# philgzl/brever

Measured on AMD Instinct MI355X. Metric: utterances/sec (4 s @16 kHz) Conv-TasNet train, higher is better.
Workload: dtype bf16

## Files before the change

brever_amd/csrc/convtasnet.hip:

```cpp
#include <hip/hip_runtime.h>
#include <stdio.h>
#include <stdlib.h>
#include <string.h>
#include <algorithm>
#include <string>
#include <vector>

#include "../../include/brever_hip.h"
#include "status.h"
#include "ctn_layout.h"
#include "gemm_rows.cuh"
#include "gemm_wgrad.cuh"
#include "gemm_ws.cuh"
#include "dwpw2_fused.cuh"
#include "gemm_wgrad_full.cuh"
#include "gemm_wgrad_full128.cuh"

constexpr int kWgSplit = 4;
#include "prep.cuh"
#include "tcn_kernels.cuh"
#include "bwd_fused.cuh"
#include "pw1_bwd.cuh"
#include "cln_kernels.cuh"

using namespace brv;

namespace {

inline long long align_up(long long x, long long a) { return (x + a - 1)/a*a; }

const brv_launch_opts kDefaultOpts = {sizeof(brv_launch_opts), 0u, 8, 0, nullptr};
thread_local const brv_launch_opts* t_opts = &kDefaultOpts;
struct OptsScope {
  const brv_launch_opts* prev;
  explicit OptsScope(const brv_launch_opts* o) : prev(t_opts) {
    t_opts = (o && o->size >= sizeof(brv_launch_opts)) ? o : &kDefaultOpts;
  }
  ~OptsScope() { t_opts = prev; }
  int check() const {
    const uint32_t unknown = t_opts->flags & ~BRV_OPT_KNOWN;
    if (!unknown) return 0;
// ... 59 lines not shown
      blk[i].p_c1_b = ptake((long long)Bnp*Hp);
      blk[i].p_rs_f = ptake((long long)rs*Hp);
      blk[i].p_rs_b = ptake((long long)Hp*rs);
      blk[i].p_c1_fp = ptake((long long)Hp*Bnp);
      blk[i].p_rs_fp = ptake((long long)rs*Hp);
      blk[i].p_rs_bp = ptake((long long)Hp*rs);
      blk[i].p_rs_g = ptake((long long)(Bnp + Scp)*Hp);
      blk[i].p_rs_gp = ptake((long long)(Bnp + Scp)*Hp);
      blk[i].p_lazy = ptake(4LL*(Bnp + Scp));
    }
    p_out_f = ptake((long long)S*Np*Scp);
    p_out_b = ptake((long long)Scp*S*Np);
    p_stamp = ptake(128);
    n_prepared = q;
    return 0;
  }
};

struct Workspace {
  long long w, x, z1, z2, skip, m, y, stats, sums, dpre, dw1, gskip, gout, eA, eB,
      e0, dwt, vg, gcopy, total;
  long long gcopy_stride, eB_stride;
  long long wgpart;
  long long h1, h2, wn, ctab, ctab_stride, cfs, cbt, ident, fake_stats, scratch_stats;
  long long vg_stride, vg_bytes;
  long long x_stride, z_stride;
  long long u, u_stride;
  long long stamp;
  long long stats_bytes;
  void init(const Layout& l, long long B, long long T) {
    long long o = 0;
    auto take = [&](long long bytes) { long long r = o; o += align_up(bytes, 256); return r; };
    const long long BT = B*T;
    w = take(BT*l.Np*2);
    x_stride = align_up(BT*l.Bnp*2, 256);
    x = take(x_stride*l.nb);
    z_stride = align_up(BT*l.Hp*2, 256);
    z1 = take(z_stride*l.nb);
    z2 = take(z_stride*l.nb);
    skip = take(BT*l.Scp*4);
    m = take(BT*l.S*l.Np*2);
    y = take(BT*l.S*l.Np*2);
    stats_bytes = (long long)(1 + 2*l.nb)*B*kStatStride*8;
    stats = take(stats_bytes);
    sums = take(stats_bytes);
    dpre = take(BT*l.S*l.Np*2);
    dw1 = take(BT*l.S*l.Np*2);
    gout = take(BT*(l.Bnp + l.Scp)*2);
    gskip = gout + (long long)l.Bnp*2;
    eA = take(BT*l.Hp*2);
    eB_stride = align_up(BT*l.Hp*2, 256);
    eB = take(eB_stride*l.nb);
    gcopy_stride = align_up(BT*l.Bnp*2, 256);
    gcopy = take(gcopy_stride*l.nb);
    e0 = take(BT*l.Np*2);
    dwt = take(BT*l.Np*2);
    vg_stride = align_up(2LL*l.N + (long long)l.nb*l.H*(5 + l.P) + 1 + 2*l.nb + 2LL*l.Hp, 64);
    vg_bytes = vg_stride*kReplicas*4;
    vg = take(vg_bytes);
    wgpart = take((long long)2*kWgSplit*l.nb*W2_G*l.H*4);
    u_stride = align_up(BT*(l.Bnp + l.Scp)*2, 256);
    u = l.fusable() ? take(u_stride*l.nb) : 0;
    stamp = take(256);
    h1 = h2 = wn = ctab = cfs = cbt = ident = fake_stats = scratch_stats = 0; ctab_stride = 0;
    if (l.causal) {
      h1 = take(z_stride*l.nb);
      h2 = take(z_stride*l.nb);
      wn = take(BT*l.Np*2);
      ctab_stride = align_up(BT*2*4, 256);
      ctab = take(ctab_stride*(1 + 2*l.nb));
      cfs = take(BT*2*4);
      cbt = take(BT*2*4);
      const long long cmax = l.Hp > l.Np ? l.Hp : l.Np;
      ident = take((2*cmax + 64)*4);
      fake_stats = take(B*kStatStride*8);
      scratch_stats = take(B*kStatStride*8);
    }
    total = o;
  }
};

struct Views {
  const Layout& l; Workspace ws; char* base; const bf16_t* prep; int B; long long T;
// ... 174 lines not shown
  if (p.Kp % GR_BK != 0 || p.Np % 64 != 0) return fail(-1, "gemm_rows: unpadded dims");
  if (p.Np % 128 == 0) return launch_gemm_rows_t<128, AK, EM>(p, batch, st);
  return launch_gemm_rows_t<64, AK, EM>(p, batch, st);
}

inline int wgrad_target(const char* label, int dflt) {
  (void)label;
  return t_opts->wg_target != 0 ? t_opts->wg_target : dflt;
}

template <int BH, int HK>
int launch_wgrad_t(WgradGroupParams& gp, hipStream_t st, int target) {
  WgradParams& p = gp.base;
  const int nprob = gp.nprob > 0 ? gp.nprob : 1;
  const int tiles = ceil_div(p.Gp, WG_BG)*(p.Hp/BH);
  const int total = p.B*ceil_div(p.T, WG_BT);
  int ns = ceil_div(target > 0 ? target : 384, tiles*nprob);
  if (target < 0) {
    int nb = p.B;
    while (tiles*nprob*nb > 2048 && nb % 2 == 0) nb /= 2;
    if (nb > ns) ns = nb;
  }
  if (ns > total) ns = total;
  if (ns < 1) ns = 1;
  p.nsplit = ns;
  dim3 grid(tiles, ns, nprob);
  hipLaunchKernelGGL((gemm_wgrad_kernel<BH, HK>), grid, dim3(256), 0, st, gp);
  BRV_HIP_OK(hipGetLastError());
  return 0;
}
template <int HK>
int launch_wgrad_group(WgradGroupParams& gp, hipStream_t st, const char* label,
                       double bytes, int target_dflt = 384) {
  const WgradParams& p = gp.base;
  if (p.T <= 0 || p.B <= 0) return 0;
  const int nprob = gp.nprob > 0 ? gp.nprob : 1;
  ProfScope prof(label, 2.0*nprob*p.B*p.T*(double)p.Gp*p.Hp, bytes*nprob, st);
  if (p.Hp % 64 != 0) return fail(-1, "wgrad: unpadded dims");
  const int target = wgrad_target(label, target_dflt);
  if (p.Hp % 128 == 0) return launch_wgrad_t<128, HK>(gp, st, target);
  return launch_wgrad_t<64, HK>(gp, st, target);
}
template <int HK>
int launch_wgrad(WgradParams& p, hipStream_t st, const char* label = "wgrad",
                 double bytes = 0, int target_dflt = 384) {
  WgradGroupParams gp;
  gp.base = p; gp.nprob = 0;
  return launch_wgrad_group<HK>(gp, st, label, bytes, target_dflt);
}

template <template <int> class F, typename... Args>
int dispatch_p(int P, Args&&... args) {
  switch (P) {
    case 1: return F<1>::run(args...);
    case 2: return F<2>::run(args...);
    case 3: return F<3>::run(args...);
    case 4: return F<4>::run(args...);
    case 5: return F<5>::run(args...);
  }
  return fail(-2, "unsupported kernel_size");
}
template <int P> struct DwFwd {
  static int run(const DwParams& p, hipStream_t st) {
    ProfScope prof("dwconv_fwd", 2.0*P*p.B*p.T*(double)p.Cp, 4.0*p.B*p.T*(double)p.Cp, st);
    dim3 grid(ceil_div(p.T, DW_TT_F)*p.B);
    hipLaunchKernelGGL((dwconv_fwd_kernel<P>), grid, dim3(256), 0, st, p);
    BRV_HIP_OK(hipGetLastError());
    return 0;
  }
};
template <int P> struct DwBwd {
// ... 49 lines not shown
  int gx = (int)((per_item + 256*8 - 1)/(256*8));
  const int cap = 1024/p.B > 1 ? 1024/p.B : 1;
  if (gx > cap) gx = cap;
  if (gx < 1) gx = 1;
  hipLaunchKernelGGL(dz_kernel, dim3(gx, p.B), dim3(256), 0, st, p);
  BRV_HIP_OK(hipGetLastError());
  return 0;
}

ASpec rows_bf16(const void* ptr, int ld, long long T) {
  ASpec a; memset(&a, 0, sizeof(a));
  a.p0 = ptr; a.ld0 = ld; a.bs0 = T*ld; a.K0 = 1 << 30; a.nsrc = 1;
  return a;
}
void set_affine(ASpec& a, const double* stats, const float* g, const float* b, int C,
                long long T) {
  a.stats = stats; a.gamma = g; a.beta = b; a.C = C;
  a.inv_n = 1.0/((double)T*(double)C); a.eps = 1e-8f;
}
ASpec frames_of(const float* wav, long long L, int hop, int K, long long stride = 0) {
  ASpec a; memset(&a, 0, sizeof(a));
  a.p0 = wav; a.hop = hop; a.Kf = K; a.wav_stride = stride > 0 ? stride : L; a.wav_len = (int)L;
  a.K0 = 1 << 30; a.nsrc = 1;
  return a;
}

struct PrepJobC { int src_off, dst_off, scale_off; unsigned short R, C, rows, cols, dst_ld, tr; };
constexpr int kPrepBatch = 168;
struct PrepBatch { PrepJobC jobs[kPrepBatch]; int n; };
static_assert(sizeof(PrepBatch) <= 4096, "kernel argument size");

struct PackJob { long long src_off, dst_off; int N, K, nsl; };
struct PackBatch { PackJob jobs[96]; int n; };
__global__ __launch_bounds__(256) void pack_frag_kernel(bf16_t* prepared, const PackBatch pb) {
  const PackJob j = pb.jobs[blockIdx.y];
  const long long total = (long long)j.N*j.K/8;
  const int KS = j.K/16;
  for (long long i = (long long)blockIdx.x*256 + threadIdx.x; i < total; i += (long long)gridDim.x*256) {
    const int n = (int)(i / (j.K/8)), k = (int)(i % (j.K/8))*8;
    const int slice = n / j.nsl, f = (n % j.nsl)/32, fr = n % 32, s = k/16, fh = (k % 16)/8;
    const long long dst = (long long)slice*j.nsl*j.K + ((long long)(f*KS + s)*64 + fr + 32*fh)*8;
    *reinterpret_cast<uint4*>(prepared + j.dst_off + dst) =
        *reinterpret_cast<const uint4*>(prepared + j.src_off + (long long)n*j.K + k);
  }
}
__global__ __launch_bounds__(256) void prep_weights_kernel(const float* params,
// ... 94 lines not shown
        float f[8];
        unpack8(q[k], f);
        const float r = rs[i + k];
#pragma unroll
        for (int j = 0; j < 8; ++j) acc[j] = __builtin_fmaf(r, f[j], acc[j]);
      }
    }
    for (; i < p.nb; ++i) {
      float f[8];
      unpack8(*reinterpret_cast<const uint4*>(src + i*p.u_stride), f);
      const float r = rs[i];
#pragma unroll
      for (int j = 0; j < 8; ++j) acc[j] = __builtin_fmaf(r, f[j], acc[j]);
    }
    float* dst = p.skip + ((long long)b*p.T + t)*p.Scp + c0;
    *reinterpret_cast<float4*>(dst) = make_float4(acc[0], acc[1], acc[2], acc[3]);
    *reinterpret_cast<float4*>(dst + 4) = make_float4(acc[4], acc[5], acc[6], acc[7]);
  }
}

}

int reduce_vector_grads(const Views& v, float* grads, hipStream_t st, int blk_lo = 0, int blk_hi = 1 << 30,
                        bool do_ln = true, bool do_tcn = true) {
  const Layout& l = v.l;
  const long long vper = (long long)l.H*(5 + l.P);
  {
    VgradParams vp; memset(&vp, 0, sizeof(vp));
    vp.vg = v.vg(); vp.grads = grads; vp.rep_stride = v.ws.vg_stride;
    vp.N = l.N; vp.H = l.H; vp.P = l.P; vp.nb = l.nb;
    vp.ln_g_off = l.ln_g; vp.blk0_off = l.blk[0].conv_w;
    vp.blk_full = l.nb > 1 ? l.blk[1].conv_w - l.blk[0].conv_w : 0;
    const BlockOff& b0 = l.blk[0];
    const BlockOff& bl = l.blk[l.nb - 1];
    vp.o_dconv_w = b0.dconv_w - b0.conv_w; vp.o_dconv_b = b0.dconv_b - b0.conv_w;
    vp.o_n1_g_full = b0.n1_g - b0.conv_w; vp.o_n1_g_last = bl.n1_g - bl.conv_w;
    vp.tcn_prelu_off = l.tcn_prelu;
    vp.blk_lo = blk_lo; vp.blk_hi = blk_hi; vp.do_ln = do_ln; vp.do_tcn = do_tcn;
    if (b0.prelu1 != b0.n1_g + 4LL*l.H || b0.prelu2 != b0.prelu1 + 1)
      return fail(-1, "vgrad_reduce: unexpected PReLU offsets");
    const long long total = 2LL*l.N + vper*l.nb + 1 + 2*l.nb;
    int gx = (int)((total + 255)/256);
    if (gx > 1024) gx = 1024;
    ProfScope prof("vgrad_reduce", 0, 4.0*total*(kReplicas + 2), st);
    hipLaunchKernelGGL(vgrad_reduce_kernel, dim3(gx), dim3(256), 0, st, vp);
    BRV_HIP_OK(hipGetLastError());
  }
  return 0;
}

__global__ void fill_identity_kernel(float* ones, float* zeros, float* one, int n,
                                     double* fake_stats, int B, double sumsq) {
  const int i = blockIdx.x*256 + threadIdx.x;
  if (i < n) { ones[i] = 1.f; zeros[i] = 0.f; }
  if (i == 0) *one = 1.f;
  if (i < B) { fake_stats[stat_sum(i)] = 0.0; fake_stats[stat_sq(i)] = sumsq; }
}

namespace {

int causal_init(const Views& v, hipStream_t st) {
  const Layout& l = v.l;
  const double sumsq = (1.0 - (double)1e-8f)*(double)v.T*(double)l.H;
  const int cmax = (int)v.cmax(), n = cmax > v.B ? cmax : v.B;
  hipLaunchKernelGGL(fill_identity_kernel, dim3((n + 255)/256), dim3(256), 0, st, v.ones(), v.zeros(),
                     v.one(), cmax, v.fake_stats(), v.B, sumsq);
  BRV_HIP_OK(hipGetLastError());
// ... 371 lines not shown
  }
  else
  if (int r = launch_wgrad_group<A_BF16>(gp, st, "pw1_wgrad", 2.0*BT*(l.Hp + l.Bnp), -1))
    return r;
  return 0;
}

int deferred_wgrads(const Views& v, const float* params, float* grads, int blk_lo, int blk_hi, hipStream_t st) {
  const Layout& l = v.l;
  const bool full_rs = l.Bnp == 128 && l.Scp == 128 && l.Hp % W2_BH == 0 && l.nb <= kWgMaxProb &&
                       !opt(BRV_OPT_NO_WGRAD_FULL);
  if (full_rs && blk_lo <= blk_hi)
    if (int r = wgrad_rs_full(v, params, grads, blk_lo, blk_hi, st)) return r;
  for (int i0 = blk_lo; i0 <= blk_hi; i0 += kWgMaxProb) {
    const int n = std::min(kWgMaxProb, blk_hi + 1 - i0);
    if (!full_rs)
      if (int r = wgrad_rs_grouped(v, params, grads, i0, n, st)) return r;
    if (int r = wgrad_pw1(v, params, grads, i0, n, st)) return r;
  }
  return 0;
}

int backward_head(const Views& v, const float* params, const float* d_out, float* grads, long long L,
                  bool bwd_fused, hipStream_t st) {
  const Layout& l = v.l; const int B = v.B; const long long T = v.T; const double BT = v.BT();
  const int BS = B*l.S, ldg = v.ldg(); GemmRowsParams g; WgradParams wg;
  if (!l.causal)
    if (int r = launch_call_init(v.sum(0), (long long)(v.ws.stats_bytes/8), v.vg(), (long long)v.ws.vg_bytes,
                                 reinterpret_cast<const int*>(v.base + v.ws.stamp), mode_stamp(l.fused_fwd()), nullptr, 0, st))
      return fail(r, "backward: call_init launch");
  memset(&g, 0, sizeof(g));
  g.a = frames_of(d_out, L, l.hop, l.K);
  g.W = v.prep + l.p_dec_b; g.T = (int)T; g.Np = l.Np; g.Kp = l.Kfp;
  g.e.out = v.dpre(); g.e.ldo = l.Np; g.e.out2 = v.dw1(); g.e.w_in = v.w(); g.e.ld_w = l.Np;
  g.e.m_in = v.m(); g.e.S = l.S;
  if (int r = launch_gemm_rows<A_FRAMES, E_MASK_BWD>(g, BS, st, "dec_bwd", 4.0*BS*L + 2.0*BT*l.Np*(1 + 3*l.S))) return r;
  memset(&wg, 0, sizeof(wg));
  wg.g = rows_bf16(v.y(), l.Np, T); wg.h = frames_of(d_out, L, l.hop, l.K);
  wg.B = BS; wg.T = (int)T; wg.Gp = l.Np; wg.Hp = l.Kfp;
  wg.out0 = grads + l.dec_w; wg.G0p = l.Np; wg.N0 = l.N; wg.Kout = l.K; wg.ldo = l.K;
  if (int r = launch_wgrad<A_FRAMES>(wg, st, "wgrad_dec", 2.0*BT*l.S*l.Np + 4.0*BS*L, l.causal ? 384 : 768)) return r;
  memset(&g, 0, sizeof(g));
  g.a = rows_bf16(v.dpre(), l.Np, T); g.a.nsrc = l.S;
  g.W = v.prep + l.p_out_b; g.T = (int)T; g.Np = l.Scp; g.Kp = l.S*l.Np;
  g.e.out = v.gskip(); g.e.ldo = ldg; g.e.src_f32 = v.skip(); g.e.ld_srcf = l.Scp;
  g.e.src_slope = params + l.tcn_prelu; g.e.dslope = v.vslope();
  g.e.rep_stride = v.ws.vg_stride; g.e.n_rep = kReplicas;
  if (int r = launch_gemm_rows<A_BF16, E_PRELU_BWD>(g, B, st, "mask_bwd", 2.0*BT*l.S*l.Np + 6.0*BT*l.Scp)) return r;
  if (bwd_fused) {
    GuDotsParams gu; memset(&gu, 0, sizeof(gu));
    gu.g = v.gskip(); gu.ldg = ldg; gu.u = v.u(l.nb - 1) + l.Bnp; gu.ldu = ldg;
    gu.v1 = reinterpret_cast<const float*>(v.prep + l.blk[l.nb - 1].p_lazy) + ldg + l.Bnp;
    gu.ncols = l.Scp; gu.B = B; gu.T = (int)T; gu.out = v.sum(2 + 2*(l.nb - 1));
    ProfScope prof("gu_dots", 0, 4.0*BT*l.Scp, st);
    int gx = (int)((T*(l.Scp/8) + 255)/256);
    if (gx > 64) gx = 64;
    hipLaunchKernelGGL(gu_dots_kernel, dim3(gx, B), dim3(256), 0, st, gu);
    BRV_HIP_OK(hipGetLastError());
  }
  for (int s = 0; s < l.S; ++s) {
    memset(&wg, 0, sizeof(wg));
    wg.g = rows_bf16(v.dpre() + (long long)s*T*l.Np, l.Np, T); wg.g.bs0 = (long long)l.S*T*l.Np;
    wg.h = rows_bf16(v.skip(), l.Scp, T); wg.h.slope = params + l.tcn_prelu;
    wg.B = B; wg.T = (int)T; wg.Gp = l.Np; wg.Hp = l.Scp;
    wg.out0 = grads + l.out_w + (long long)s*l.N*l.Sc; wg.G0p = l.Np; wg.N0 = l.N;
    wg.Kout = l.Sc; wg.ldo = l.Sc; wg.gbias0 = grads + l.out_b + (long long)s*l.N;
    if (int r = launch_wgrad<A_F32>(wg, st, "wgrad_out", 2.0*BT*l.Np + 4.0*BT*l.Scp, l.causal ? 384 : 256)) return r;
  }
  return 0;
}

int backward_block_dw(const Views& v, const float* params, int i, bool bwd_fused, hipStream_t st) {
  const Layout& l = v.l; const int B = v.B; const long long T = v.T; const double BT = v.BT();
  const int ldg = v.ldg(); GemmRowsParams g;
  const BlockOff& b = l.blk[i];
  const bool has_res = i < l.nb - 1;
  const int dil = 1 << (i % l.layers);
  const int rs0 = has_res ? l.Bnp : 0;
  const bool blk_fused = bwd_fused && (((l.P - 1)*dil)/2) % dil == 0;
  if (!blk_fused) {
    memset(&g, 0, sizeof(g));
    g.a = rows_bf16(has_res ? v.gout() : v.gskip(), ldg, T);
    g.W = v.prep + b.p_rs_b; g.T = (int)T; g.Np = l.Hp; g.Kp = rs0 + l.Scp;
    g.Wp = v.prep + b.p_rs_bp; g.wp_nsl = 32;
    g.e.out = v.eA(); g.e.ldo = l.Hp; g.e.N = l.H;
    g.e.src = v.z2(i); g.e.ld_src = l.Hp; g.e.src_slope = params + b.prelu2;
    g.e.src_stats = v.stat(2 + 2*i); g.e.inv_n = 1.0/((double)T*l.H); g.e.eps = 1e-8f;
    g.e.gamma = params + b.n2_g;
    g.e.dgamma = v.vslot(i) + 2*l.H; g.e.dbeta = v.vslot(i) + 3*l.H;
    g.e.rep_stride = v.ws.vg_stride; g.e.n_rep = kReplicas;
// ... 94 lines not shown
  g.e.out2 = i > 0 ? v.gcopy(i - 1) : nullptr; g.e.ld_srcf = l.Bnp;
  if (bwd_fused && i > 0) {
    g.e.gu_u = v.u(i - 1); g.e.ld_gu = ldg; g.e.gu_gskip = v.gskip(); g.e.ld_gs = ldg;
    g.e.gu_v1 = reinterpret_cast<const float*>(v.prep + l.blk[i - 1].p_lazy) + ldg;
    g.e.gu_out = v.sum(2 + 2*(i - 1));
  }
  if (fuse_dz1 && l.pw1_rc()) return backward_block_pw1_rc(v, params, i, g.e, bwd_fused, st);
  if (fuse_dz1) {
    g.a.p1 = v.z1(i); g.a.ld1 = l.Hp; g.a.bs1 = T*l.Hp;
    g.a.slope = params + b.prelu1; g.a.stats = v.stat(1 + 2*i); g.a.sums = v.sum(1 + 2*i);
    g.a.inv_n = 1.0/((double)T*l.H); g.a.eps = 1e-8f; g.a.C = l.H;
    g.e.dslope = v.vslope() + 1 + 2*i; g.e.rep_stride = v.ws.vg_stride; g.e.n_rep = kReplicas;
    return launch_gemm_rows<A_DZ, E_ADD>(g, B, st, "pw1_dgrad", 2.0*BT*(3*l.Hp + l.Bnp*(has_res ? 2 : 1)));
  }
  return launch_gemm_rows<A_BF16, E_ADD>(g, B, st, "pw1_dgrad", 2.0*BT*(l.Hp + l.Bnp*(has_res ? 2 : 1)));
}

int backward_block(const Views& v, const float* params, int i, bool bwd_fused, hipStream_t st) {
  if (int r = backward_block_dw(v, params, i, bwd_fused, st)) return r;
  return backward_block_pw1(v, params, i, bwd_fused, st);
}

int backward_tail(const Views& v, const float* params, const float* wave, long long wave_stride, float* grads,
                  long long L, hipStream_t st) {
  const Layout& l = v.l; const int B = v.B; const long long T = v.T; const double BT = v.BT();
  const int ldg = v.ldg(); GemmRowsParams g; WgradParams wg;
  memset(&g, 0, sizeof(g));
  g.a = rows_bf16(v.gout(), ldg, T);
  g.W = v.prep + l.p_bott_b; g.T = (int)T; g.Np = l.Np; g.Kp = l.Bnp;
  g.e.out = v.e0(); g.e.ldo = l.Np; g.e.N = l.N;
  g.e.src = v.w(); g.e.ld_src = l.Np; g.e.src_stats = v.stat(0);
  g.e.inv_n = 1.0/((double)T*l.N); g.e.eps = 1e-8f;
  g.e.gamma = params + l.ln_g; g.e.dgamma = v.vg(); g.e.dbeta = v.vg() + l.N;
  g.e.rep_stride = v.ws.vg_stride; g.e.n_rep = kReplicas;
  g.e.sums_out = v.sum(0);
  if (int r = launch_gemm_rows<A_BF16, E_GLN_BWD>(g, B, st, "bottleneck_dgrad", 2.0*BT*(l.Bnp + 2*l.Np))) return r;
  memset(&wg, 0, sizeof(wg));
  wg.g = rows_bf16(v.gout(), ldg, T); wg.h = rows_bf16(v.w(), l.Np, T);
  set_affine(wg.h, v.stat(0), params + l.ln_g, params + l.ln_b, l.N, T);
  wg.B = B; wg.T = (int)T; wg.Gp = l.Bnp; wg.Hp = l.Np;
  wg.out0 = grads + l.bott_w; wg.G0p = l.Bnp; wg.N0 = l.Bn; wg.Kout = l.N; wg.ldo = l.N;
  wg.gbias0 = grads + l.bott_b;
  if (int r = launch_wgrad<A_BF16>(wg, st, "bottleneck_wgrad", 2.0*BT*(l.Bnp + l.Np), 256)) return r;
  CombineParams cb; memset(&cb, 0, sizeof(cb));
  cb.e0 = v.e0(); cb.w = v.w(); cb.dw1 = v.dw1(); cb.dw = v.dwt(); cb.B = B; cb.T = (int)T;
  cb.Cp = l.Np; cb.C = l.N; cb.S = l.S; cb.stats = v.stat(0); cb.sums = v.sum(0);
  cb.inv_n = 1.0/((double)T*l.N); cb.eps = 1e-8f;
  {
    const long long per_item = T*(l.Np/8);
    int gx = (int)((per_item + 1023)/1024);
    if (gx > 2048) gx = 2048;
    if (gx < 1) gx = 1;
    ProfScope prof("gln0_bwd", 0, 2.0*BT*l.Np*(3 + l.S), st);
    hipLaunchKernelGGL(gln0_bwd_combine_kernel, dim3(gx, B), dim3(256), 0, st, cb);
    BRV_HIP_OK(hipGetLastError());
  }
  memset(&wg, 0, sizeof(wg));
  wg.g = rows_bf16(v.dwt(), l.Np, T); wg.h = frames_of(wave, L, l.hop, l.K, wave_stride);
  wg.B = B; wg.T = (int)T; wg.Gp = l.Np; wg.Hp = l.Kfp;
  wg.out0 = grads + l.enc_w; wg.G0p = l.Np; wg.N0 = l.N; wg.Kout = l.K; wg.ldo = l.K;
  if (int r = launch_wgrad<A_FRAMES>(wg, st, "wgrad_enc", 2.0*BT*l.Np + 4.0*B*L, 768)) return r;
  return 0;
}

int backward_causal_block(const Views& v, const float* params, float* grads, int i, hipStream_t st) {
  const Layout& l = v.l; const int B = v.B; const long long T = v.T; const double BT = v.BT();
  const int ldg = v.ldg(); GemmRowsParams g; WgradParams wg;
  const BlockOff& b = l.blk[i];
  const bool has_res = i < l.nb - 1;
  const int dil = 1 << (i % l.layers);
  const int rs0 = has_res ? l.Bnp : 0;
  memset(&wg, 0, sizeof(wg));
  wg.g = rows_bf16(has_res ? v.gout() : v.gskip(), ldg, T);
  wg.h = rows_bf16(v.h2(i), l.Hp, T);
  wg.B = B; wg.T = (int)T; wg.Gp = rs0 + l.Scp; wg.Hp = l.Hp;
  wg.out0 = has_res ? grads + b.res_w : nullptr; wg.out1 = grads + b.skip_w;
  wg.G0p = rs0; wg.N0 = has_res ? l.Bn : 0; wg.N1 = l.Sc; wg.Kout = l.H; wg.ldo = l.H;
  wg.gbias0 = has_res ? grads + b.res_b : nullptr; wg.gbias1 = grads + b.skip_b;
  if (int r = launch_wgrad<A_BF16>(wg, st, "pw2_wgrad", 2.0*BT*(rs0 + l.Scp + l.Hp))) return r;
  memset(&g, 0, sizeof(g));
  g.a = rows_bf16(has_res ? v.gout() : v.gskip(), ldg, T);
  g.W = v.prep + b.p_rs_b; g.T = (int)T; g.Np = l.Hp; g.Kp = rs0 + l.Scp;
  g.e.out = v.eA(); g.e.ldo = l.Hp; g.e.N = l.H;
  if (int r = launch_gemm_rows<A_BF16, E_STORE>(g, B, st, "pw2_dgrad", 2.0*BT*(rs0 + l.Scp + l.Hp))) return r;
// ... 35 lines not shown
  wg.B = B; wg.T = (int)T; wg.Gp = l.Bnp; wg.Hp = l.Np;
  wg.out0 = grads + l.bott_w; wg.G0p = l.Bnp; wg.N0 = l.Bn; wg.Kout = l.N; wg.ldo = l.N;
  wg.gbias0 = grads + l.bott_b;
  if (int r = launch_wgrad<A_BF16>(wg, st, "bottleneck_wgrad", 2.0*BT*(l.Bnp + l.Np))) return r;
  memset(&g, 0, sizeof(g));
  g.a = rows_bf16(v.gout(), ldg, T);
  g.W = v.prep + l.p_bott_b; g.T = (int)T; g.Np = l.Np; g.Kp = l.Bnp;
  g.e.out = v.e0(); g.e.ldo = l.Np; g.e.N = l.N;
  if (int r = launch_gemm_rows<A_BF16, E_STORE>(g, B, st, "bottleneck_dgrad", 2.0*BT*(l.Bnp + l.Np))) return r;
  if (int r = cln_backward(v, v.e0(), v.w(), nullptr, params + l.ln_g, v.tab(0), v.dwt(), v.dw1(), l.S, v.vg(),
                           v.vg() + l.N, nullptr, v.ws.vg_stride, B, T, l.Np, l.N, st)) return r;
  memset(&wg, 0, sizeof(wg));
  wg.g = rows_bf16(v.dwt(), l.Np, T); wg.h = frames_of(wave, L, l.hop, l.K, wave_stride);
  wg.B = B; wg.T = (int)T; wg.Gp = l.Np; wg.Hp = l.Kfp;
  wg.out0 = grads + l.enc_w; wg.G0p = l.Np; wg.N0 = l.N; wg.Kout = l.K; wg.ldo = l.K;
  if (int r = launch_wgrad<A_FRAMES>(wg, st, "wgrad_enc", 2.0*BT*l.Np + 4.0*B*L)) return r;
  return reduce_vector_grads(v, grads, st);
}

int backward_causal(const Views& v, const float* params, const float* wave, long long wave_stride,
                    const float* d_out, float* grads, long long L, hipStream_t st) {
  if (int r = causal_init(v, st)) return r;
  BRV_HIP_OK(hipMemsetAsync(v.vg(), 0, v.ws.vg_bytes, st));
  if (int r = backward_head(v, params, d_out, grads, L, false, st)) return r;
  for (int i = v.l.nb - 1; i >= 0; --i)
    if (int r = backward_causal_block(v, params, grads, i, st)) return r;
  return backward_causal_tail(v, params, wave, wave_stride, grads, L, st);
}

}

extern "C" {

#ifdef BRV_DIAG
int brv_debug_read(long long* out, int64_t n) {
  (void)hipDeviceSynchronize();
  const int r = (int)hipMemcpy(out, debug_buffer(), (size_t)n*8, hipMemcpyDeviceToHost);
  (void)hipMemset(debug_buffer(), 0, 1 << 20);
  return r;
}
#endif

void* brv_prof_create(int by_dilation) {
  Prof* p = new Prof();
  p->by_dil = by_dilation != 0;
  return p;
}
// ... 241 lines not shown

int brv_ctn_backward_part(const brv_ctn_config* cfg, const float* params, const void* prepared,
                          void* workspace, const float* wave, int64_t wave_stride, const float* d_out,
                          float* grads,
                          int64_t batch, int64_t length, int32_t part, int32_t nparts,
                          const brv_launch_opts* opts, brv_stream_t stream) {
  OptsScope scope(opts);
  if (int r = scope.check()) return r;
  Layout l; if (int r = l.init(cfg)) return r;
  hipStream_t st = (hipStream_t)stream;
  const int B = (int)batch; const long long L = length;
  const long long T = l.frames(L);
  if (B < 1 || T < 1) return fail(-1, "empty batch or input shorter than one frame");
  if (nparts < 1 || part < 0 || part >= nparts) return fail(-1, "bad part");
  const Views v(l, workspace, prepared, B, T);
  if (l.causal) {
    if (part != nparts - 1) return 0;
    return backward_causal(v, params, wave, wave_stride, d_out, grads, L, st);
  }
  int blk_lo, blk_hi; part_range(l.nb, part, nparts, blk_lo, blk_hi);
  const bool head = part == 0, tail = part == nparts - 1;
  const bool bwd_fused = l.fused_fwd() && bwd_fuse_requested() && l.Bnp == 128 && l.Scp == 128 &&
                         l.Hp % HL_CG == 0 && !opt(BRV_OPT_NO_DZ_FUSE) && bf_frames_ok(T);
  if (head)
    if (int r = backward_head(v, params, d_out, grads, L, bwd_fused, st)) return r;
  for (int i = blk_hi; i >= blk_lo; --i)
    if (int r = backward_block(v, params, i, bwd_fused, st)) return r;
  if (int r = deferred_wgrads(v, params, grads, blk_lo, blk_hi, st)) return r;
  if (tail)
    if (int r = backward_tail(v, params, wave, wave_stride, grads, L, st)) return r;
  return reduce_vector_grads(v, grads, st, blk_lo, blk_hi, tail, head);
}

}
```

brever_amd/csrc/gemm_rows.cuh:

```cuda
#pragma once
#include "common.cuh"

namespace brv {

enum AKind { A_BF16 = 0, A_F32 = 1, A_FRAMES = 2, A_DZ = 3 };
enum EMode {
  E_STORE = 0,
  E_RES_SKIP = 1,
  E_MASK = 2,
  E_OLA = 3,
  E_GLN_BWD = 4,
  E_ADD = 5,
  E_MASK_BWD = 6,
  E_PRELU_BWD = 7
};

struct ASpec {
  const void* p0; const void* p1;
  int ld0, ld1;
  long long bs0, bs1;
  int K0;
  int nsrc;
  int hop, Kf; long long wav_stride; int wav_len;
  const float* slope;
  const double* stats;
  const float* gamma; const float* beta; int C;
  double inv_n; float eps;
  const double* sums;
  void* xout; const float* lazy_v0; const float* lazy_v1;
  void* z2out; const float* taps; const float* dbias; const float* slope2; double* stats2_out;
  int dil, left;
};

struct EpiSpec {
  void* out; int ldo;
  const float* bias; const float* bias2; int N, Nsplit, N2;
  double* stats_out; const float* stats_slope;
  const bf16_t* res_in; int ld_res; float* skip; int ld_skip; int skip_init;
  const bf16_t* w_in; int ld_w; bf16_t* m_out; int S; int Np_src;
  float* wave_out; int hop, Kf; long long wave_stride; int wave_len;
  const bf16_t* src; int ld_src; const float* src_slope; const double* src_stats;
  double inv_n; float eps;
  const float* gamma; float* dgamma; float* dbeta; double* sums_out;
  long long rep_stride; int n_rep;
  const bf16_t* add_in; int ld_add;
  const bf16_t* m_in; bf16_t* out2;
// ... 1 lines not shown
  const bf16_t* gu_u; int ld_gu; const bf16_t* gu_gskip; int ld_gs; const float* gu_v1; double* gu_out;
};

struct GemmRowsParams {
  ASpec a;
  const bf16_t* W;
  const bf16_t* Wp;
  int wp_nsl;
  int T, Np, Kp;
  int n_ttiles, n_ntiles, batch;
#ifdef BRV_DIAG
  int dbg;
  long long* dbg_out;
#endif
  EpiSpec e;
};

__device__ __forceinline__ int xcd_remap(int id, int nwg) {
  const int xcd = id & 7, slot = id >> 3;
  const int q = nwg >> 3, r = nwg & 7;
  return (xcd < r ? xcd*(q + 1) : r*(q + 1) + (xcd - r)*q) + slot;
}

constexpr int GR_BM = 128;
constexpr int GR_BK = 64;
constexpr int GR_LDS_K = GR_BK + 8;

template <int BN>
struct GemmRowsSmem {
  static constexpr int kMain = (GR_BM + BN)*GR_LDS_K*2;
  static constexpr int kLdc = BN + 4;
  static constexpr int kEpi = GR_BM*kLdc*4;
  static constexpr int kBytes = kMain > kEpi ? kMain : kEpi;
};

template <int BN, int AK, int EM>
__global__ __launch_bounds__(256) void gemm_rows_kernel(const GemmRowsParams p) {
  __shared__ __attribute__((aligned(16))) unsigned char smem[GemmRowsSmem<BN>::kBytes];
  bf16_t* As = reinterpret_cast<bf16_t*>(smem);
  bf16_t* Ws = As + GR_BM*GR_LDS_K;
  float* Cs = reinterpret_cast<float*>(smem);
  constexpr int LDC = GemmRowsSmem<BN>::kLdc;
  constexpr int NT = BN/32;
  constexpr int WCH = BN/32;

  const int tid = threadIdx.x;
// ... 11 lines not shown
  const ASpec& a = p.a;

  NormStat ns = {0.f, 1.f};
  const bool affine = AK != A_DZ && a.stats != nullptr;
  if (a.stats != nullptr) ns = norm_stat(a.stats, b, a.inv_n, a.eps);
  const float slope = a.slope ? *a.slope : 1.f;
  const bool has_prelu = AK != A_DZ && a.slope != nullptr;
  float dz_m1 = 0.f, dz_m2 = 0.f, dz_da = 0.f;
  if (AK == A_DZ) {
    dz_m1 = (float)(a.sums[stat_sum(b)]*a.inv_n);
    dz_m2 = (float)(a.sums[stat_sq(b)]*a.inv_n);
  }
  uint4 araw_z[(AK == A_DZ) ? 4 : 1];

  uint4 araw_b[4];
  float araw_f[(AK == A_BF16) ? 1 : 4][8];
  float asc[8], ash[8];
  uint4 wraw[WCH];

  auto load_tile = [&](int kt) {
    const int kbase = kt*GR_BK + kc*8;
    if (AK == A_FRAMES) {
      const float* wav = reinterpret_cast<const float*>(a.p0) + (long long)b*a.wav_stride;
#pragma unroll
      for (int ci = 0; ci < 4; ++ci) {
        const int t = t0 + arow + 32*ci;
#pragma unroll
        for (int j = 0; j < 8; ++j) {
          const int k = kbase + j;
          const long long idx = (long long)t*a.hop + k;
          float v = 0.f;
          if (t < T && k < a.Kf && idx < a.wav_len) v = wav[idx];
          araw_f[(AK == A_BF16) ? 0 : ci][j] = v;
        }
      }
    } else {
      bool first = kbase < a.K0;
      int ld = first ? a.ld0 : a.ld1;
      int kk = first ? kbase : kbase - a.K0;
      long long boff = (long long)b*(first ? a.bs0 : a.bs1);
      if (a.nsrc > 1) {
        first = true; ld = a.ld0;
        const int s = kbase / a.ld0;
        kk = kbase - s*a.ld0;
        boff = ((long long)b*a.nsrc + s)*a.bs0;
      }
#pragma unroll
      for (int ci = 0; ci < 4; ++ci) {
        const int t = t0 + arow + 32*ci;
        const long long off = boff + (long long)t*ld + kk;
        if (AK == A_DZ) {
          const long long o0 = (long long)b*a.bs0 + (long long)t*a.ld0 + kbase;
          const long long o1 = (long long)b*a.bs1 + (long long)t*a.ld1 + kbase;
          araw_b[ci] = (t < T) ? *reinterpret_cast<const uint4*>(reinterpret_cast<const bf16_t*>(a.p0) + o0)
                               : make_uint4(0, 0, 0, 0);
          araw_z[(AK == A_DZ) ? ci : 0] =
// ... 378 lines not shown
```

brever_amd/csrc/gemm_wgrad.cuh:

```cuda
#pragma once
#include "gemm_rows.cuh"
#include "gfx950.cuh"

namespace brv {

struct WgradParams {
  ASpec g;
  ASpec h;
  int B, T;
  int Gp, Hp;
  float* out0; float* out1; int G0p;
  int N0, N1;
  int Kout, ldo;
  float* gbias0; float* gbias1;
  int nsplit;
};

constexpr int kWgMaxProb = 24;
struct WgradProb {
  const void* g0; const void* g1; const void* h;
  float* out0; float* out1; float* gbias0; float* gbias1;
  const float* slope; const double* stats; const float* gamma; const float* beta;
};
struct WgradGroupParams {
  WgradParams base;
  int nprob;
  WgradProb prob[kWgMaxProb];
};

constexpr int WG_BT = 64;
constexpr int WG_BG = 128;

typedef __attribute__((ext_vector_type(8))) short s16x8;

__device__ __forceinline__ bf16x8 tr_frag(const bf16_t* tile, int ld, int row0,
                                          int col0, int lane) {
  const int g4 = lane >> 4, i = lane & 15, q = i >> 2, pp = i & 3;
  const int col = col0 + 16*(g4 & 1) + 4*pp;
  const int row = row0 + 8*(g4 >> 1) + q;
// ... 69 lines not shown
  const bool h_aff = H.stats != nullptr;
  const bool h_prelu = H.slope != nullptr;
  const float hslope = h_prelu ? *H.slope : 1.f;
  float hg[8], hb[8];
  load8_masked(h_aff ? H.gamma : nullptr, hch, H.C, hg);
  load8_masked(h_aff ? H.beta : nullptr, hch, H.C, hb);

  uint4 graw[4];
  uint4 hraw_b[HCH];
  float hraw_f[(HK == A_BF16) ? 1 : HCH][8];
  float bias_acc[8];
#pragma unroll
  for (int j = 0; j < 8; ++j) bias_acc[j] = 0.f;

  auto load_chunk = [&](int c) {
    const int b = c / cpi, t0 = (c % cpi)*WG_BT;
#pragma unroll
    for (int ci = 0; ci < 4; ++ci) {
      const int t = t0 + grow + 16*ci;
      graw[ci] = (g_ok && t < T)
          ? *reinterpret_cast<const uint4*>(gsrc + (long long)b*gbs + (long long)t*gld + gk)
          : make_uint4(0, 0, 0, 0);
    }
#pragma unroll
    for (int ci = 0; ci < HCH; ++ci) {
      const int t = t0 + hrow + HRS*ci;
      if (HK == A_BF16) {
        hraw_b[ci] = (h_ok && t < T)
            ? *reinterpret_cast<const uint4*>(reinterpret_cast<const bf16_t*>(H.p0)
                                              + (long long)b*H.bs0 + (long long)t*H.ld0 + hch)
            : make_uint4(0, 0, 0, 0);
      } else if (HK == A_F32) {
        float4 lo = make_float4(0, 0, 0, 0), hi = lo;
        if (h_ok && t < T) {
          const float* s = reinterpret_cast<const float*>(H.p0) + (long long)b*H.bs0 + (long long)t*H.ld0 + hch;
          lo = *reinterpret_cast<const float4*>(s);
          hi = *reinterpret_cast<const float4*>(s + 4);
        }
        float* d = hraw_f[(HK == A_BF16) ? 0 : ci];
        d[0] = lo.x; d[1] = lo.y; d[2] = lo.z; d[3] = lo.w;
        d[4] = hi.x; d[5] = hi.y; d[6] = hi.z; d[7] = hi.w;
      } else {
        const float* wav = reinterpret_cast<const float*>(H.p0) + (long long)b*H.wav_stride;
#pragma unroll
        for (int j = 0; j < 8; ++j) {
          const int k = hch + j;
// ... 55 lines not shown
#pragma unroll
  for (int j = 0; j < NT; ++j)
#pragma unroll
    for (int i = 0; i < 16; ++i) acc[j][i] = 0.f;

  if (c_begin < c_end) load_chunk(c_begin);
  for (int c = c_begin; c < c_end; ++c) {
    __syncthreads();
    store_chunk(c);
    __syncthreads();
    if (c + 1 < c_end) load_chunk(c + 1);
#pragma unroll
    for (int s = 0; s < WG_BT/16; ++s) {
      const bf16x8 af = tr_frag(Gs, LDG, 16*s, 32*wid, lane);
#pragma unroll
      for (int j = 0; j < NT; ++j) {
        const bf16x8 bfr = tr_frag(Hs, LDH, 16*s, 32*j, lane);
        acc[j] = __builtin_amdgcn_mfma_f32_32x32x16_bf16(af, bfr, acc[j], 0, 0, 0);
      }
    }
  }

  const int fr = lane & 31, fh = lane >> 5;
#pragma unroll
  for (int j = 0; j < NT; ++j) {
    const int k = k0 + 32*j + fr;
#pragma unroll
    for (int i = 0; i < 16; ++i) {
      const int n = n0 + 32*wid + (i & 3) + 8*(i >> 2) + 4*fh;
      if (k < p.Kout) {
        if (n < p.G0p) {
          if (n < p.N0) atomic_add_f32(p.out0 + (long long)n*p.ldo + k, acc[j][i]);
        } else {
          const int n1 = n - p.G0p;
          if (n1 < p.N1) atomic_add_f32(p.out1 + (long long)n1*p.ldo + k, acc[j][i]);
        }
      }
    }
  }
  if ((p.gbias0 || p.gbias1) && htile == 0) {
    __syncthreads();
    float* sc = reinterpret_cast<float*>(Gs);
#pragma unroll
    for (int j = 0; j < 8; ++j) sc[grow*WG_BG + gcc*8 + j] = bias_acc[j];
    __syncthreads();
    if (tid < WG_BG) {
// ... 11 lines not shown
```

brever_amd/csrc/tcn_kernels.cuh:

```cuda
#pragma once
#include "common.cuh"

namespace brv {

struct DwParams {
  const bf16_t* z1;
  bf16_t* z2;
  const bf16_t* dz2;
  bf16_t* e1;
  int B, T, Cp, C;
  const float* slope1; const double* stats1; const float* gamma1; const float* beta1;
  double inv_n; float eps;
  const float* taps;
  const float* bias;
  int dil, left;
  double* stats2; const float* slope2;
  float* dgamma1; float* dbeta1; float* dtaps; float* dbias; double* sums1;
  long long rep_stride;
  const bf16_t* z2in; const double* sums2; float* dslope2;
};

constexpr int kReplicas = 64;

#ifndef BRV_DW_NB
// ... 512 lines not shown
  reduce_cols(dbia, p.dbias, 1, 0);
#pragma unroll
  for (int k = 0; k < P; ++k) reduce_cols(dtap[k], p.dtaps, P, k);
  const double tot1 = block_sum((double)l1, dscr);
  const double tot2 = block_sum((double)l2, dscr + 8);
  if (tid == 0) {
    atomic_add_f64(p.sums1 + stat_sum(b), tot1);
    atomic_add_f64(p.sums1 + stat_sq(b), tot2);
  }
  __syncthreads();
  const float sa = block_sum(da2, red);
  if (tid == 0) atomic_add_f32(p.dslope2 + (long long)(blockIdx.x % kReplicas)*p.rep_stride, sa);
}

struct VgradParams {
  const float* vg; float* grads; long long rep_stride;
  int N, H, P, nb;
  long long ln_g_off;
  long long blk0_off;
  long long blk_full;
  long long o_dconv_w, o_dconv_b, o_n1_g_full, o_n1_g_last;
  long long tcn_prelu_off;
  int blk_lo, blk_hi, do_ln, do_tcn;
};
__global__ __launch_bounds__(256) void vgrad_reduce_kernel(const VgradParams p) {
  const long long per_blk = (long long)p.H*(5 + p.P);
  const long long n_vec = 2LL*p.N + per_blk*p.nb;
  const long long total = n_vec + 1 + 2*p.nb;
  for (long long i = (long long)blockIdx.x*256 + threadIdx.x; i < total;
       i += (long long)gridDim.x*256) {
    long long dst;
    if (i >= n_vec) {
      const int k = (int)(i - n_vec);
      if (k == 0) { if (!p.do_tcn) continue; dst = p.tcn_prelu_off; }
      else {
        const int blk = (k - 1) >> 1;
        if (blk < p.blk_lo || blk > p.blk_hi) continue;
        const long long n1 = blk == p.nb - 1 ? p.o_n1_g_last : p.o_n1_g_full;
        dst = p.blk0_off + blk*p.blk_full + n1 + 4LL*p.H + ((k - 1) & 1);
      }
    } else if (i < 2LL*p.N) {
      if (!p.do_ln) continue;
      dst = p.ln_g_off + i;
    } else {
      const long long j = i - 2LL*p.N;
      const int blk = (int)(j / per_blk);
      if (blk < p.blk_lo || blk > p.blk_hi) continue;
      const long long k = j % per_blk;
// ... 55 lines not shown
```

Baseline: 2470.

## Replace atomic wgrad accumulation for leaf weights with split partials reduced in vgrad kernel

For the non-causal path, the decoder, encoder, output and bottleneck weight-gradient GEMMs now write per-split partial sums into dedicated workspace buffers instead of doing float atomics into the gradient arrays. Those partials are summed later inside the existing vector-gradient reduce kernel, and the split counts and targets are capped. This is meant to remove atomic contention and allow more splits. It also adds vectorized float4/float2 loads for gathering waveform frames when the pointer, stride and hop are aligned. In exchange it uses extra workspace and memory traffic for the partials and adds work to the reduce kernel.

```diff
diff --git a/brever_amd/csrc/convtasnet.hip b/brever_amd/csrc/convtasnet.hip
--- a/brever_amd/csrc/convtasnet.hip
+++ b/brever_amd/csrc/convtasnet.hip
@@ -17,6 +17,8 @@
 #include "gemm_wgrad_full128.cuh"
 
 constexpr int kWgSplit = 4;
+constexpr int kLeafSplitFrames = 192, kLeafSplitRows = 64;
+constexpr int kLeafTargetFrames = 4*kLeafSplitFrames, kLeafTargetRows = 4*kLeafSplitRows;
 #include "prep.cuh"
 #include "tcn_kernels.cuh"
 #include "bwd_fused.cuh"
@@ -122,6 +124,8 @@
       e0, dwt, vg, gcopy, total;
   long long gcopy_stride, eB_stride;
   long long wgpart;
+  long long leaf_dec, leaf_enc, leaf_out, leaf_out_stride, leaf_bott;
+  int leaf_f, leaf_r;
   long long h1, h2, wn, ctab, ctab_stride, cfs, cbt, ident, fake_stats, scratch_stats;
   long long vg_stride, vg_bytes;
   long long x_stride, z_stride;
@@ -159,6 +163,17 @@
     vg_bytes = vg_stride*kReplicas*4;
     vg = take(vg_bytes);
     wgpart = take((long long)2*kWgSplit*l.nb*W2_G*l.H*4);
+    leaf_dec = leaf_enc = leaf_out = leaf_bott = 0; leaf_out_stride = 0; leaf_f = leaf_r = 0;
+    if (!l.causal) {
+      const long long chunks = B*((T + WG_BT - 1)/WG_BT);
+      leaf_f = (int)std::min<long long>(kLeafSplitFrames, chunks);
+      leaf_r = (int)std::min<long long>(kLeafSplitRows, chunks);
+      leaf_dec = take(4LL*leaf_f*l.Np*l.K);
+      leaf_enc = take(4LL*leaf_f*l.Np*l.K);
+      leaf_out_stride = align_up(4LL*leaf_r*l.Np*(l.Sc + 1), 256);
+      leaf_out = take(leaf_out_stride*l.S);
+      leaf_bott = take(4LL*leaf_r*l.Bnp*(l.N + 1));
+    }
     u_stride = align_up(BT*(l.Bnp + l.Scp)*2, 256);
     u = l.fusable() ? take(u_stride*l.nb) : 0;
     stamp = take(256);
@@ -379,6 +394,7 @@
     if (nb > ns) ns = nb;
   }
   if (ns > total) ns = total;
+  if (p.part && ns > p.part_splits) ns = p.part_splits;
   if (ns < 1) ns = 1;
   p.nsplit = ns;
   dim3 grid(tiles, ns, nprob);
@@ -403,7 +419,25 @@
                  double bytes = 0, int target_dflt = 384) {
   WgradGroupParams gp;
   gp.base = p; gp.nprob = 0;
-  return launch_wgrad_group<HK>(gp, st, label, bytes, target_dflt);
+  const int r = launch_wgrad_group<HK>(gp, st, label, bytes, target_dflt);
+  p.nsplit = gp.base.nsplit;
+  return r;
+}
+template <int HK>
+int launch_wgrad_leaf(WgradParams& p, float* part, int splits, LeafJobs* jobs, hipStream_t st, const char* label,
+                      double bytes, int target_dflt) {
+  const bool room = jobs && splits > 0 && jobs->n < kMaxLeafJobs && p.out1 == nullptr && p.G0p == p.Gp;
+  if (room) {
+    p.part = part; p.part_splits = splits;
+    p.part_bias = p.gbias0 ? part + (long long)splits*p.Gp*p.Kout : nullptr;
+  }
+  if (int r = launch_wgrad<HK>(p, st, label, bytes, target_dflt)) return r;
+  if (room && p.T > 0 && p.B > 0) {
+    LeafJob& j = jobs->job[jobs->n++];
+    j.part = p.part; j.part_bias = p.part_bias; j.out = p.out0; j.bias_out = p.part_bias ? p.gbias0 : nullptr;
+    j.ns = p.nsplit; j.Gp = p.Gp; j.Hp = p.Hp; j.N = p.N0; j.K = p.Kout; j.ldo = p.ldo;
+  }
+  return 0;
 }
 
 template <template <int> class F, typename... Args>
@@ -499,6 +533,10 @@
   ASpec a; memset(&a, 0, sizeof(a));
   a.p0 = wav; a.hop = hop; a.Kf = K; a.wav_stride = stride > 0 ? stride : L; a.wav_len = (int)L;
   a.K0 = 1 << 30; a.nsrc = 1;
+  const auto aligned = [&](int w) {
+    return reinterpret_cast<unsigned long long>(wav) % (4ull*w) == 0 && a.wav_stride % w == 0 && hop % w == 0;
+  };
+  a.wav_vec = L < 8 ? 1 : aligned(4) ? 4 : aligned(2) ? 2 : 1;
   return a;
 }
 
@@ -639,7 +677,7 @@
 }
 
 int reduce_vector_grads(const Views& v, float* grads, hipStream_t st, int blk_lo = 0, int blk_hi = 1 << 30,
-                        bool do_ln = true, bool do_tcn = true) {
+                        bool do_ln = true, bool do_tcn = true, const LeafJobs* leaf = nullptr) {
   const Layout& l = v.l;
   const long long vper = (long long)l.H*(5 + l.P);
   {
@@ -657,9 +695,17 @@
     if (b0.prelu1 != b0.n1_g + 4LL*l.H || b0.prelu2 != b0.prelu1 + 1)
       return fail(-1, "vgrad_reduce: unexpected PReLU offsets");
     const long long total = 2LL*l.N + vper*l.nb + 1 + 2*l.nb;
-    int gx = (int)((total + 255)/256);
+    int leaf_wgs = 0; double leaf_bytes = 0;
+    if (leaf) {
+      vp.leaf = *leaf;
+      for (int q = 0; q < leaf->n; ++q) {
+        leaf_wgs += leaf_blocks(leaf->job[q]);
+        leaf_bytes += 4.0*256*leaf_blocks(leaf->job[q])*(leaf->job[q].ns + 2);
+      }
+    }
+    int gx = std::max((int)((total + 255)/256), leaf_wgs);
     if (gx > 1024) gx = 1024;
-    ProfScope prof("vgrad_reduce", 0, 4.0*total*(kReplicas + 2), st);
+    ProfScope prof("vgrad_reduce", 0, 4.0*total*(kReplicas + 2) + leaf_bytes, st);
     hipLaunchKernelGGL(vgrad_reduce_kernel, dim3(gx), dim3(256), 0, st, vp);
     BRV_HIP_OK(hipGetLastError());
   }
@@ -1077,7 +1123,7 @@
 }
 
 int backward_head(const Views& v, const float* params, const float* d_out, float* grads, long long L,
-                  bool bwd_fused, hipStream_t st) {
+                  bool bwd_fused, LeafJobs* leaf, hipStream_t st) {
   const Layout& l = v.l; const int B = v.B; const long long T = v.T; const double BT = v.BT();
   const int BS = B*l.S, ldg = v.ldg(); GemmRowsParams g; WgradParams wg;
   if (!l.causal)
@@ -1094,7 +1140,8 @@
   wg.g = rows_bf16(v.y(), l.Np, T); wg.h = frames_of(d_out, L, l.hop, l.K);
   wg.B = BS; wg.T = (int)T; wg.Gp = l.Np; wg.Hp = l.Kfp;
   wg.out0 = grads + l.dec_w; wg.G0p = l.Np; wg.N0 = l.N; wg.Kout = l.K; wg.ldo = l.K;
-  if (int r = launch_wgrad<A_FRAMES>(wg, st, "wgrad_dec", 2.0*BT*l.S*l.Np + 4.0*BS*L, l.causal ? 384 : 768)) return r;
+  if (int r = launch_wgrad_leaf<A_FRAMES>(wg, v.f32(v.ws.leaf_dec), v.ws.leaf_f, leaf, st, "wgrad_dec",
+                                          2.0*BT*l.S*l.Np + 4.0*BS*L, l.causal ? 384 : kLeafTargetFrames)) return r;
   memset(&g, 0, sizeof(g));
   g.a = rows_bf16(v.dpre(), l.Np, T); g.a.nsrc = l.S;
   g.W = v.prep + l.p_out_b; g.T = (int)T; g.Np = l.Scp; g.Kp = l.S*l.Np;
@@ -1120,7 +1167,8 @@
     wg.B = B; wg.T = (int)T; wg.Gp = l.Np; wg.Hp = l.Scp;
     wg.out0 = grads + l.out_w + (long long)s*l.N*l.Sc; wg.G0p = l.Np; wg.N0 = l.N;
     wg.Kout = l.Sc; wg.ldo = l.Sc; wg.gbias0 = grads + l.out_b + (long long)s*l.N;
-    if (int r = launch_wgrad<A_F32>(wg, st, "wgrad_out", 2.0*BT*l.Np + 4.0*BT*l.Scp, l.causal ? 384 : 256)) return r;
+    if (int r = launch_wgrad_leaf<A_F32>(wg, v.f32(v.ws.leaf_out + v.ws.leaf_out_stride*s), v.ws.leaf_r, leaf, st, "wgrad_out",
+                                         2.0*BT*l.Np + 4.0*BT*l.Scp, l.causal ? 384 : kLeafTargetRows)) return r;
   }
   return 0;
 }
@@ -1261,7 +1309,7 @@
 }
 
 int backward_tail(const Views& v, const float* params, const float* wave, long long wave_stride, float* grads,
-                  long long L, hipStream_t st) {
+                  long long L, LeafJobs* leaf, hipStream_t st) {
   const Layout& l = v.l; const int B = v.B; const long long T = v.T; const double BT = v.BT();
   const int ldg = v.ldg(); GemmRowsParams g; WgradParams wg;
   memset(&g, 0, sizeof(g));
@@ -1280,7 +1328,8 @@
   wg.B = B; wg.T = (int)T; wg.Gp = l.Bnp; wg.Hp = l.Np;
   wg.out0 = grads + l.bott_w; wg.G0p = l.Bnp; wg.N0 = l.Bn; wg.Kout = l.N; wg.ldo = l.N;
   wg.gbias0 = grads + l.bott_b;
-  if (int r = launch_wgrad<A_BF16>(wg, st, "bottleneck_wgrad", 2.0*BT*(l.Bnp + l.Np), 256)) return r;
+  if (int r = launch_wgrad_leaf<A_BF16>(wg, v.f32(v.ws.leaf_bott), v.ws.leaf_r, leaf, st, "bottleneck_wgrad",
+                                        2.0*BT*(l.Bnp + l.Np), kLeafTargetRows)) return r;
   CombineParams cb; memset(&cb, 0, sizeof(cb));
   cb.e0 = v.e0(); cb.w = v.w(); cb.dw1 = v.dw1(); cb.dw = v.dwt(); cb.B = B; cb.T = (int)T;
   cb.Cp = l.Np; cb.C = l.N; cb.S = l.S; cb.stats = v.stat(0); cb.sums = v.sum(0);
@@ -1298,7 +1347,8 @@
   wg.g = rows_bf16(v.dwt(), l.Np, T); wg.h = frames_of(wave, L, l.hop, l.K, wave_stride);
   wg.B = B; wg.T = (int)T; wg.Gp = l.Np; wg.Hp = l.Kfp;
   wg.out0 = grads + l.enc_w; wg.G0p = l.Np; wg.N0 = l.N; wg.Kout = l.K; wg.ldo = l.K;
-  if (int r = launch_wgrad<A_FRAMES>(wg, st, "wgrad_enc", 2.0*BT*l.Np + 4.0*B*L, 768)) return r;
+  if (int r = launch_wgrad_leaf<A_FRAMES>(wg, v.f32(v.ws.leaf_enc), v.ws.leaf_f, leaf, st, "wgrad_enc",
+                                          2.0*BT*l.Np + 4.0*B*L, kLeafTargetFrames)) return r;
   return 0;
 }
 
@@ -1380,7 +1430,7 @@
                     const float* d_out, float* grads, long long L, hipStream_t st) {
   if (int r = causal_init(v, st)) return r;
   BRV_HIP_OK(hipMemsetAsync(v.vg(), 0, v.ws.vg_bytes, st));
-  if (int r = backward_head(v, params, d_out, grads, L, false, st)) return r;
+  if (int r = backward_head(v, params, d_out, grads, L, false, nullptr, st)) return r;
   for (int i = v.l.nb - 1; i >= 0; --i)
     if (int r = backward_causal_block(v, params, grads, i, st)) return r;
   return backward_causal_tail(v, params, wave, wave_stride, grads, L, st);
@@ -1668,14 +1718,15 @@
   const bool head = part == 0, tail = part == nparts - 1;
   const bool bwd_fused = l.fused_fwd() && bwd_fuse_requested() && l.Bnp == 128 && l.Scp == 128 &&
                          l.Hp % HL_CG == 0 && !opt(BRV_OPT_NO_DZ_FUSE) && bf_frames_ok(T);
+  LeafJobs leaf; leaf.n = 0;
   if (head)
-    if (int r = backward_head(v, params, d_out, grads, L, bwd_fused, st)) return r;
+    if (int r = backward_head(v, params, d_out, grads, L, bwd_fused, &leaf, st)) return r;
   for (int i = blk_hi; i >= blk_lo; --i)
     if (int r = backward_block(v, params, i, bwd_fused, st)) return r;
   if (int r = deferred_wgrads(v, params, grads, blk_lo, blk_hi, st)) return r;
   if (tail)
-    if (int r = backward_tail(v, params, wave, wave_stride, grads, L, st)) return r;
-  return reduce_vector_grads(v, grads, st, blk_lo, blk_hi, tail, head);
-}
-
-}
+    if (int r = backward_tail(v, params, wave, wave_stride, grads, L, &leaf, st)) return r;
+  return reduce_vector_grads(v, grads, st, blk_lo, blk_hi, tail, head, &leaf);
+}
+
+}
diff --git a/brever_amd/csrc/gemm_rows.cuh b/brever_amd/csrc/gemm_rows.cuh
--- a/brever_amd/csrc/gemm_rows.cuh
+++ b/brever_amd/csrc/gemm_rows.cuh
@@ -22,6 +22,7 @@
   int K0;
   int nsrc;
   int hop, Kf; long long wav_stride; int wav_len;
+  int wav_vec;
   const float* slope;
   const double* stats;
   const float* gamma; const float* beta; int C;
@@ -69,6 +70,52 @@
   return (xcd < r ? xcd*(q + 1) : r*(q + 1) + (xcd - r)*q) + slot;
 }
 
+template <int NR, int W>
+__device__ __forceinline__ void frames_gather(const ASpec& a, const float* wav, int t0, int tstep, int T, int k0,
+                                              float (*out)[8]) {
+  static_assert(W == 4 || W == 2, "vector width in floats");
+  bool whole[NR];
+#pragma unroll
+  for (int ci = 0; ci < NR; ++ci) {
+    whole[ci] = false;
+#pragma unroll
+    for (int j = 0; j < 8; ++j) out[ci][j] = 0.f;
+  }
+  if (k0 >= a.Kf) return;
+#pragma unroll
+  for (int ci = 0; ci < NR; ++ci) {
+    const int t = t0 + ci*tstep;
+    const long long idx = (long long)t*a.hop + k0;
+    whole[ci] = t < T && k0 + 8 <= a.Kf && idx + 8 <= (long long)a.wav_len;
+    const float* s = wav + (whole[ci] ? idx : 0LL);
+    if (W == 4) {
+      const float4 lo = *reinterpret_cast<const float4*>(s);
+      const float4 hi = *reinterpret_cast<const float4*>(s + 4);
+      out[ci][0] = lo.x; out[ci][1] = lo.y; out[ci][2] = lo.z; out[ci][3] = lo.w;
+      out[ci][4] = hi.x; out[ci][5] = hi.y; out[ci][6] = hi.z; out[ci][7] = hi.w;
+    } else {
+#pragma unroll
+      for (int q = 0; q < 4; ++q) {
+        const float2 v = *reinterpret_cast<const float2*>(s + 2*q);
+        out[ci][2*q] = v.x; out[ci][2*q + 1] = v.y;
+      }
+    }
+  }
+#pragma unroll
+  for (int ci = 0; ci < NR; ++ci) {
+    if (whole[ci]) continue;
+    const int t = t0 + ci*tstep;
+#pragma unroll
+    for (int j = 0; j < 8; ++j) {
+      const int k = k0 + j;
+      const long long idx = (long long)t*a.hop + k;
+      float v = 0.f;
+      if (t < T && k < a.Kf && idx < a.wav_len) v = wav[idx];
+      out[ci][j] = v;
+    }
+  }
+}
+
 constexpr int GR_BM = 128;
 constexpr int GR_BK = 64;
 constexpr int GR_LDS_K = GR_BK + 8;
@@ -126,16 +173,23 @@
     const int kbase = kt*GR_BK + kc*8;
     if (AK == A_FRAMES) {
       const float* wav = reinterpret_cast<const float*>(a.p0) + (long long)b*a.wav_stride;
-#pragma unroll
-      for (int ci = 0; ci < 4; ++ci) {
-        const int t = t0 + arow + 32*ci;
-#pragma unroll
-        for (int j = 0; j < 8; ++j) {
-          const int k = kbase + j;
-          const long long idx = (long long)t*a.hop + k;
-          float v = 0.f;
-          if (t < T && k < a.Kf && idx < a.wav_len) v = wav[idx];
-          araw_f[(AK == A_BF16) ? 0 : ci][j] = v;
+      constexpr int NRA = (AK == A_BF16) ? 1 : 4;
+      if (a.wav_vec == 4) {
+        frames_gather<NRA, 4>(a, wav, t0 + arow, 32, T, kbase, araw_f);
+      } else if (a.wav_vec == 2) {
+        frames_gather<NRA, 2>(a, wav, t0 + arow, 32, T, kbase, araw_f);
+      } else {
+#pragma unroll
+        for (int ci = 0; ci < 4; ++ci) {
+          const int t = t0 + arow + 32*ci;
+#pragma unroll
+          for (int j = 0; j < 8; ++j) {
+            const int k = kbase + j;
+            const long long idx = (long long)t*a.hop + k;
+            float v = 0.f;
+            if (t < T && k < a.Kf && idx < a.wav_len) v = wav[idx];
+            araw_f[(AK == A_BF16) ? 0 : ci][j] = v;
+          }
         }
       }
     } else {
diff --git a/brever_amd/csrc/gemm_wgrad.cuh b/brever_amd/csrc/gemm_wgrad.cuh
--- a/brever_amd/csrc/gemm_wgrad.cuh
+++ b/brever_amd/csrc/gemm_wgrad.cuh
@@ -14,7 +14,48 @@
   int Kout, ldo;
   float* gbias0; float* gbias1;
   int nsplit;
+  float* part; float* part_bias; int part_splits;
 };
+
+struct LeafJob {
+  const float* part; const float* part_bias; float* out; float* bias_out;
+  int ns, Gp, Hp, N, K, ldo;
+};
+constexpr int kMaxLeafJobs = 8;
+struct LeafJobs { int n; LeafJob job[kMaxLeafJobs]; };
+
+__host__ __device__ inline int leaf_blocks(const LeafJob& J) {
+  return (int)(((long long)J.Gp*(J.K + (J.bias_out ? 1 : 0)) + 255)/256);
+}
+__device__ __forceinline__ void leaf_reduce(const LeafJobs& jobs) {
+  int total = 0;
+  for (int q = 0; q < jobs.n; ++q) total += leaf_blocks(jobs.job[q]);
+  for (int blk = blockIdx.x; blk < total; blk += gridDim.x) {
+    int q = 0, local = blk;
+    for (; q < jobs.n - 1 && local >= leaf_blocks(jobs.job[q]); ++q) local -= leaf_blocks(jobs.job[q]);
+    const LeafJob& J = jobs.job[q];
+    const long long rows = (long long)J.K*J.Gp, tile = rows;
+    const long long e = (long long)local*256 + threadIdx.x;
+    const bool is_bias = e >= rows;
+    if (e >= rows + (J.bias_out ? J.Gp : 0)) continue;
+    const int n = (int)(is_bias ? e - rows : e % J.Gp), k = (int)(is_bias ? 0 : e / J.Gp);
+    if (n >= J.N) continue;
+    const float* src = is_bias ? J.part_bias + n : J.part + e;
+    const long long stride = is_bias ? J.Gp : tile;
+    float s = 0.f;
+    int i = 0;
+    for (; i + 16 <= J.ns; i += 16) {
+      float v[16];
+#pragma unroll
+      for (int u = 0; u < 16; ++u) v[u] = src[(i + u)*stride];
+#pragma unroll
+      for (int u = 0; u < 16; ++u) s += v[u];
+    }
+    for (; i < J.ns; ++i) s += src[i*stride];
+    float* dst = is_bias ? J.bias_out + n : J.out + (long long)n*J.ldo + k;
+    *dst += s;
+  }
+}
 
 constexpr int kWgMaxProb = 24;
 struct WgradProb {
@@ -130,6 +171,13 @@
           ? *reinterpret_cast<const uint4*>(gsrc + (long long)b*gbs + (long long)t*gld + gk)
           : make_uint4(0, 0, 0, 0);
     }
+    if (HK == A_FRAMES && H.wav_vec >= 2) {
+      constexpr int NRH = (HK == A_BF16) ? 1 : HCH;
+      const float* wav = reinterpret_cast<const float*>(H.p0) + (long long)b*H.wav_stride;
+      if (H.wav_vec == 4) frames_gather<NRH, 4>(H, wav, t0 + hrow, HRS, T, hch, hraw_f);
+      else frames_gather<NRH, 2>(H, wav, t0 + hrow, HRS, T, hch, hraw_f);
+      return;
+    }
 #pragma unroll
     for (int ci = 0; ci < HCH; ++ci) {
       const int t = t0 + hrow + HRS*ci;
@@ -231,6 +279,33 @@
   }
 
   const int fr = lane & 31, fh = lane >> 5;
+  if (p.part) {
+    float* dst = p.part + (long long)by*p.Kout*p.Gp;
+#pragma unroll
+    for (int j = 0; j < NT; ++j) {
+      const int k = k0 + 32*j + fr;
+#pragma unroll
+      for (int g = 0; g < 4; ++g) {
+        const int n = n0 + 32*wid + 8*g + 4*fh;
+        if (n < p.Gp && k < p.Kout)
+          *reinterpret_cast<float4*>(dst + (long long)k*p.Gp + n) =
+              make_float4(acc[j][4*g], acc[j][4*g + 1], acc[j][4*g + 2], acc[j][4*g + 3]);
+      }
+    }
+    if (p.part_bias && htile == 0) {
+      __syncthreads();
+      float* sc = reinterpret_cast<float*>(Gs);
+#pragma unroll
+      for (int j = 0; j < 8; ++j) sc[grow*WG_BG + gcc*8 + j] = bias_acc[j];
+      __syncthreads();
+      if (tid < WG_BG && n0 + tid < p.Gp) {
+        float s = 0.f;
+        for (int r = 0; r < 16; ++r) s += sc[r*WG_BG + tid];
+        p.part_bias[(long long)by*p.Gp + n0 + tid] = s;
+      }
+    }
+    return;
+  }
 #pragma unroll
   for (int j = 0; j < NT; ++j) {
     const int k = k0 + 32*j + fr;
diff --git a/brever_amd/csrc/tcn_kernels.cuh b/brever_amd/csrc/tcn_kernels.cuh
--- a/brever_amd/csrc/tcn_kernels.cuh
+++ b/brever_amd/csrc/tcn_kernels.cuh
@@ -1,5 +1,6 @@
 #pragma once
 #include "common.cuh"
+#include "gemm_wgrad.cuh"
 
 namespace brv {
 
@@ -558,8 +559,10 @@
   long long o_dconv_w, o_dconv_b, o_n1_g_full, o_n1_g_last;
   long long tcn_prelu_off;
   int blk_lo, blk_hi, do_ln, do_tcn;
+  LeafJobs leaf;
 };
 __global__ __launch_bounds__(256) void vgrad_reduce_kernel(const VgradParams p) {
+  leaf_reduce(p.leaf);
   const long long per_blk = (long long)p.H*(5 + p.P);
   const long long n_vec = 2LL*p.N + per_blk*p.nb;
   const long long total = n_vec + 1 + 2*p.nb;
```

After: 2491, median of 4. Within noise of the previous version (+0.9%).
